# krea-ai/realtime-video

Measured on AMD Instinct MI355X. Metric: frames/sec at 832x480, 4-step 14B T2V (per-step DiT latency in config), higher is better.
Workload: dtype bf16

## Files before the change

### __graft_entry__.py

```python
import os
import sys

ROOT = os.path.dirname(os.path.abspath(__file__))
if ROOT not in sys.path:
    sys.path.insert(0, ROOT)


def build() -> None:
    from realtime_video_amd import _lib
    _lib.build(verbose=False)
    import realtime_video_amd.attention
    import realtime_video_amd.causal_model
    import realtime_video_amd.pipeline
    import realtime_video_amd.session
    import realtime_video_amd.taehv
    import realtime_video_amd.vae_decoder
    lib = _lib.load()
    missing = [s for s in _lib.declared_symbols() if not hasattr(lib, s)]
    if missing:
        raise RuntimeError(f"librtv_hip.so lacks symbols declared in include/rtv_hip.h: {missing}")
    import re
    import subprocess
    def audit(script, *argv, **env):
        r = subprocess.run([os.path.join(ROOT, "scripts", "micro", script), *argv], capture_output=True, text=True,
                           env=dict(os.environ, **env))
        return r.stdout + ("\n[stderr]\n" + r.stderr if r.stderr.strip() else "") + (f"\n[exit {r.returncode}]" if r.returncode else "")

    out = audit("w4_audit.sh", "600", W4_AUDIT_DIR=os.path.join(ROOT, "realtime_video_amd", "csrc", "build", "w4_audit"))
    ok = all(re.search(pat, out) for pat in (r"accumulation register outside asm: 0\b", r"v_accvgpr outside asm: 0\b", r"\bscratch 0\b",
                                              r"vgpr_spill_count: 0\b", r"private_segment_fixed_size: 0\b"))
    if not ok:
        raise RuntimeError("attn_w4 audit failed (scripts/micro/w4_audit.sh):\n" + out)
    out = audit("g5_audit.sh", G5_AUDIT_DIR=os.path.join(ROOT, "realtime_video_amd", "csrc", "build", "g5_audit"))
    if len(re.findall(r"AUDIT gemm5 F16=\d: vgpr_spills 0 private_segment 0 scratch_ops 0 mfma 120 compiler_acc_refs_before_last_accumulator_read 0 ", out)) != 2:
        raise RuntimeError("gemm5 audit failed (scripts/micro/g5_audit.sh):\n" + out)
    out = audit("h4_audit.sh", H4_AUDIT_DIR=os.path.join(ROOT, "realtime_video_amd", "csrc", "build", "h4_audit"))
    if len(re.findall(r"AUDIT _ZN3rtv1[78]conv_halo4p?_kernel\S*: arch_vgprs \d+ vgpr_spills 0 sgpr_spills \d+ private_segment 0 scratch_ops 0 "
                      r"mfma 216 compiler_acc_refs 0 \(a0-a7: 0\)", out)) != 2:
        raise RuntimeError("conv_halo4 audit failed (scripts/micro/h4_audit.sh):\n" + out)
    print(f"build ok: {_lib.LIB_PATH} ({len(_lib.declared_symbols())} C-ABI symbols; attn_w4 / gemm5 / conv_halo4 register audits clean)")


def smoke() -> None:
    import torch
    from oracle import vae_oracle as vo
    from oracle import wan_oracle as wo
    from realtime_video_amd.causal_model import CausalWanModel
# ... 46 lines not shown
```

### include/rtv_hip_lab.h

```cpp
#ifndef RTV_HIP_LAB_H
#define RTV_HIP_LAB_H
#ifdef __cplusplus
extern "C" {
#endif

int rtv_attn_set_waves(int waves);

int rtv_gemm_set_half_tail(int on);
int rtv_gemm_set_ragged_strips(int on);
int rtv_gemm_set_skip_idle(int on);
int rtv_conv_set_fuse_norm(int on);
int rtv_attn_set_skip_idle(int on);
int rtv_conv_set_halo(int on);
int rtv_dit_set_direct_v(int on);
int rtv_rope_set_wave(int mode);
int rtv_vae_set_fresh_tap_skip(int on);
int rtv_lab_build(void);

#ifdef __cplusplus
}
#endif
#endif
```

### realtime_video_amd/_lib.py

```python
import ctypes
import os
import subprocess

_HERE = os.path.dirname(os.path.abspath(__file__))
LIB_PATH = os.environ.get("RTV_LIB_PATH") or os.path.join(_HERE, "librtv_hip.so")
CSRC = os.path.join(_HERE, "csrc")

ABI_VERSION = 103

_lib = None

c_int, c_i64, c_f32, c_vp = ctypes.c_int, ctypes.c_int64, ctypes.c_float, ctypes.c_void_p

SIGNATURES = {
    "rtv_version": [],
    "rtv_quantize_fp8": [c_vp, c_i64, c_int, c_int, c_vp, c_i64, c_vp, c_vp, c_vp],
    "rtv_gemm_fp8": [c_vp, c_int, c_vp, c_int, c_vp, c_f32, c_vp, c_int, c_int, c_int, c_int, c_vp, c_int, c_vp, c_int,
                     c_int, c_int, c_vp, c_int, c_vp],
    "rtv_prof_enable": [c_int],
    "rtv_prof_read": [c_int, ctypes.POINTER(ctypes.c_double), ctypes.POINTER(c_i64),
                      ctypes.POINTER(ctypes.c_double)],
    "rtv_prof_reset": [],
    "rtv_prof_set_stride": [c_int, c_int],
    "rtv_prof_read_seen": [c_int, ctypes.POINTER(c_i64), ctypes.POINTER(ctypes.c_double)],
    "rtv_prof_bracket_overhead": [c_int, c_vp, ctypes.POINTER(ctypes.c_double)],
    "rtv_attn_fwd": [c_vp, c_vp, c_vp, c_vp, c_int, c_int, c_int, c_int, c_int,
                     c_i64, c_i64, c_i64, c_i64, c_i64, c_i64, c_i64, c_i64,
                     c_f32, c_int, c_int, c_int, c_vp],
    "rtv_attn_fwd_win": [c_vp, c_vp, c_vp, c_vp, c_int, c_int, c_int, c_int, c_int, c_int, c_int,
                         c_i64, c_i64, c_i64, c_i64, c_i64, c_i64, c_i64, c_i64,
                         c_f32, c_int, c_int, c_int, c_vp],
    "rtv_attn_fwd_dup": [c_vp, c_vp, c_vp, c_vp, c_int, c_int, c_int, c_int, c_int,
                         c_i64, c_i64, c_i64, c_i64, c_i64, c_i64, c_i64, c_i64,
                         c_f32, c_int, c_int, c_int, c_vp],
    "rtv_attn_fwd_split": [c_vp, c_vp, c_vp, c_vp, c_int, c_int, c_int, c_int, c_int, c_int, c_int,
                           c_i64, c_i64, c_i64, c_i64, c_i64, c_i64, c_i64, c_i64,
                           c_f32, c_int, c_int, c_int, c_vp, ctypes.c_size_t, c_int, c_vp],
    "rtv_attn_set_waves": [c_int],
    "rtv_attn_set_skip_idle": [c_int],
    "rtv_gemm_set_half_tail": [c_int],
    "rtv_gemm_set_skip_idle": [c_int],
    "rtv_gemm_set_ragged_strips": [c_int],
    "rtv_lab_build": [],
    "rtv_rope_set_wave": [c_int],
    "rtv_gemm": [c_vp, c_int, c_vp, c_int, c_vp, c_int, c_int, c_int, c_int,
                 c_vp, c_int, c_vp, c_int, c_int, c_int, c_vp, c_int, c_int, c_int, c_vp],
    "rtv_layernorm_modulate": [c_vp, c_vp, c_int, c_int, c_f32, c_vp, c_vp, c_int, c_int, c_int, c_vp, c_vp, c_vp],
    "rtv_rmsnorm": [c_vp, c_int, c_vp, c_int, c_int, c_int, c_f32, c_vp, c_vp],
    "rtv_qk_norm_rope_cache": [c_vp, c_vp, c_vp, c_vp, c_i64, c_int, c_int, c_int, c_int, c_f32,
                               c_vp, c_vp, c_vp, c_int, c_int, c_int, c_int, c_int, c_vp],
    "rtv_qk_norm_rope_cache_ring": [c_vp, c_vp, c_vp, c_vp, c_i64, c_int, c_int, c_int, c_int, c_f32,
                                    c_vp, c_vp, c_vp, c_int, c_int, c_int, c_int, c_int, c_int, c_int, c_int, c_vp],
    "rtv_modulation_table": [c_vp, c_vp, c_vp, c_int, c_int, c_int, c_int, c_int, c_vp],
    "rtv_sinusoidal_embedding": [c_vp, c_vp, c_int, c_int, c_vp],
# ... 79 lines not shown
```

### realtime_video_amd/csrc/attn_common.h

```cpp
#pragma once
#include "rtv_common.h"
#include "rtv_internal.h"

namespace rtv {

struct AttnParams {
  const uint16_t* q;
  const uint16_t* k;
  const uint16_t* v;
  uint16_t* o;
  int B, Lq, Lkv, H;
  int64_t q_bs, q_rs, k_bs, k_rs, v_bs, v_rs, o_bs, o_rs;
  float scale_log2e;
  int causal_block, q_offset;
  int n_qtiles;
  int n0, delta;
  int off0;
  int skip_idle;
  int dup_key;
  float dup_bias;
  int kv_splits;
  float* part_o;
  float* part_ml;
};

constexpr int ATT_D = 128;
constexpr int ATT_QW = 32;
constexpr int ATT_KT = 64;
constexpr int ATT_TILE_BYTES = ATT_KT * ATT_D * 2;

template <int V>
struct IntC {
  static constexpr int value = V;
};

template <bool F16>
// ... 76 lines not shown
```

### realtime_video_amd/csrc/attn_fwd.hip

```cpp
#include "attn_common.h"

namespace rtv {

#ifdef RTV_ATTN_TRACE
__device__ unsigned* g_attn_trace = nullptr;
#define ATT_STAMP(i)                                                                    \
  do {                                                                                  \
    if (tr_on && j >= 20 && j < 24) {                                                   \
      __builtin_amdgcn_sched_barrier(0);                                                \
      const unsigned t_ = (unsigned)__builtin_readcyclecounter();                       \
      if (lane == 0) tr_dst[(j - 20) * 6 + (i)] = t_;                                   \
      __builtin_amdgcn_sched_barrier(0);                                                \
    }                                                                                   \
  } while (0)
#else
#define ATT_STAMP(i)
#endif

template <bool F16>
__global__ __launch_bounds__(256) void attn_combine_kernel(const float* __restrict__ part_o, const float* __restrict__ part_ml,
                                                           uint16_t* __restrict__ o, int S, int B, int H, int Lq, int64_t o_bs,
                                                           int64_t o_rs) {
  const int64_t nrows = (int64_t)B * H * Lq;
  const int64_t row = (int64_t)blockIdx.x * 16 + (threadIdx.x >> 4);
// ... 583 lines not shown

using namespace rtv;

#ifdef RTV_ATTN_TRACE
extern "C" int rtv_attn_debug_trace(unsigned* buf) {
  return hipMemcpyToSymbol(HIP_SYMBOL(rtv::g_attn_trace), &buf, sizeof(buf)) == hipSuccess ? 0 : -1;
}
#endif

static std::atomic<int> g_attn_waves{0};
static std::atomic<bool> g_attn_lockstep{false};
static std::atomic<bool> g_attn_force_pp{false};
static std::atomic<bool> g_attn_skip_idle{true};
static std::atomic<int> g_attn_w4{-2};
constexpr int W4_DEFAULT = 600;
namespace rtv {
int launch_attn_w4(const AttnParams& p, bool f16, int variant, dim3 grid, hipStream_t stream);
}

extern "C" int rtv_attn_set_skip_idle(int on) {
  g_attn_skip_idle = on != 0;
  return 0;
}

extern "C" int rtv_attn_set_waves(int waves) {
  if (waves != 0 && waves != 4 && waves != 8 && waves != 81 && waves != 82 && !(waves >= 840 && waves <= 1639))
    return set_error(-1, "attn_set_waves: 0 (auto), 4, 8, 81 (256 rows, lockstep schedule), 82 (256 rows, four-phase schedule) or "
                         "840 + v (256 rows, one wave per SIMD, kernel variant v: attn_w4.hip)");
  g_attn_lockstep = waves == 81;
  g_attn_force_pp = waves == 82;
  g_attn_w4 = waves >= 840 ? waves - 840 : (waves == 81 || waves == 82 ? -1 : -2);
  g_attn_waves = waves > 8 ? 8 : waves;
// ... 96 lines not shown
  if (kv_splits > (Lkv + ATT_KT - 1) / ATT_KT) kv_splits = (Lkv + ATT_KT - 1) / ATT_KT;
  if (kv_splits < 1) kv_splits = 1;
  p.kv_splits = kv_splits;
  p.part_o = nullptr;
  p.part_ml = nullptr;
  if (kv_splits > 1) {
    if (dup_key >= 0) return set_error(-1, "attn_fwd: no KV split of a window with a counted key");
    const size_t rows = (size_t)kv_splits * B * H * Lq;
    if (!split_ws || ((uintptr_t)split_ws & 15) || split_ws_bytes < rows * (ATT_D + 2) * sizeof(float))
      return set_error(-1, "attn_fwd: split workspace missing, misaligned or too small (rtv_attn_split_workspace_bytes)");
    p.part_o = (float*)split_ws;
    p.part_ml = p.part_o + rows * ATT_D;
  }
  p.causal_block = causal_block;
  p.q_offset = q_offset;
  p.n0 = Lkv1 > 0 ? Lkv0 : Lkv;
  p.delta = Lkv1 > 0 ? seg1_row - Lkv0 : 0;
  int waves = g_attn_waves;
  const int cus = device_num_cus() > 0 ? device_num_cus() : 256;
  if (waves == 0) waves = ((int64_t)B * H * ((Lq + 255) / 256) * kv_splits < (int64_t)cus * 5 / 8 || Lkv <= 512) ? 4 : 8;
  const int qt_rows = ATT_QW * waves;
  p.n_qtiles = (Lq + qt_rows - 1) / qt_rows;
  const int lds = 4 * ATT_TILE_BYTES;
  const bool f16 = dtype == RTV_DTYPE_F16;
  const void* kerns[4] = {(const void*)attn_fwd_kernel<false, 8>, (const void*)attn_fwd_kernel<true, 8>,
                          (const void*)attn_fwd_kernel<false, 4>, (const void*)attn_fwd_kernel<true, 4>};
  static LdsAttr lds_attr[4];
  const int ki = (waves == 4 ? 2 : 0) + (f16 ? 1 : 0);
  if (int st = ensure_dynamic_lds(kerns[ki], lds, &lds_attr[ki], "attn_fwd")) return st;
  const int grid = B * H * p.n_qtiles;
// ... 19 lines not shown
    note_kernel(DK_ATTN_SPLIT_COMBINE);
    if (f16) hipLaunchKernelGGL((attn_combine_kernel<true>), cg, ct, 0, (hipStream_t)stream, p.part_o, p.part_ml, p.o, kv_splits, B, H, Lq, p.o_bs, p.o_rs);
    else hipLaunchKernelGGL((attn_combine_kernel<false>), cg, ct, 0, (hipStream_t)stream, p.part_o, p.part_ml, p.o, kv_splits, B, H, Lq, p.o_bs, p.o_rs);
    return check_launch("attn_combine");
  };
  p.off0 = 0;
  p.skip_idle = g_attn_skip_idle ? 1 : 0;
  const int base_shift = (Lkv1 > 0 && seg1_row < 0) ? seg1_row : 0;
  const int64_t top0 = (int64_t)p.n0 - base_shift, top1 = (int64_t)Lkv + p.delta - base_shift;
  const int64_t rs_max = k_row_stride > v_row_stride ? k_row_stride : v_row_stride;
  const bool offsets_fit = k_row_stride > 0 && v_row_stride > 0 &&
                           ((top0 > top1 ? top0 : top1) + ATT_KT) * rs_max * 2 < 0x7fffffffLL;
  int w4v = g_attn_w4;
  if (w4v == -2) w4v = Lkv >= 1024 ? W4_DEFAULT : -1;
  if (waves == 8 && w4v >= 0 && !f16 && Lkv1 == 0 && dup_key < 0 && offsets_fit) {
    if (int st = launch_attn_w4(p, f16, w4v, g, (hipStream_t)stream)) return st;
    note_kernel(DK_ATTN_W4);
    if (kv_splits > 1) return combine();
    return check_launch("attn_w4");
  }
  if (waves == 8 && !g_attn_lockstep && offsets_fit && dup_key < 0 && (Lkv >= 1024 || g_attn_force_pp)) {
    p.k += (int64_t)base_shift * k_row_stride;
    p.v += (int64_t)base_shift * v_row_stride;
    p.off0 = -base_shift;
    p.delta -= base_shift;
#ifdef RTV_ATTN_TRACE
    const int lds_pp = 2 * ATT_NB * ATT_TILE_BYTES + 256;
#else
    const int lds_pp = 2 * ATT_NB * ATT_TILE_BYTES;
#endif
    static LdsAttr pp_attr[2];
    const void* kp = f16 ? (const void*)attn_fwd_pp_kernel<true> : (const void*)attn_fwd_pp_kernel<false>;
// ... 19 lines not shown
```

### realtime_video_amd/csrc/attn_w4.hip

```cpp
#include "attn_common.h"

namespace rtv {
namespace w4 {

constexpr int NSLOT = 4;
constexpr int LDS_BYTES = 2 * NSLOT * ATT_TILE_BYTES;
constexpr int V_BASE = NSLOT * ATT_TILE_BYTES;
constexpr int QT = 256;
constexpr int QW = 64;

enum OpKind { OP_MAX = 0, OP_CMB, OP_XCH0, OP_XCH1, OP_DEC, OP_F, OP_E, OP_A, OP_CV, OP_SUM };
struct Op {
  int kind, qb, idx, sub, cost;
};
constexpr int N_PAIRS = 32;
constexpr int MAX_OPS = 300;
struct OpTable {
  Op op[MAX_OPS];
  int n;
};
template <bool RS>
constexpr OpTable make_ops() {
  OpTable t{};
  int n = 0;
// ... 169 lines not shown
  asm volatile("v_accvgpr_read_b32 %0, a[%c1]" : "=v"(r) : "n"(SRC));
  return r;
}
template <int REG>
__device__ __forceinline__ void acc_scale(float f) {
  float t;
  asm volatile("v_accvgpr_read_b32 %0, a[%c2]\n\ts_nop 0\n\tv_mul_f32 %0, %0, %1\n\ts_nop 0\n\tv_accvgpr_write_b32 a[%c2], %0" : "=&v"(t) : "v"(f), "n"(REG));
}
__device__ __forceinline__ void acc_settle() { asm volatile("s_nop 15\n\ts_nop 7" ); }

}

#ifdef RTV_LAB
__device__ unsigned long long* g_w4_probe = nullptr;
#endif

template <bool F16, int VARL>
__global__ __launch_bounds__(256, 1) void attn_fwd_w4_kernel(AttnParams p) {
  using namespace w4;
  constexpr int VAR = VARL % 10, LAB = (VARL / 10) % 10, OPT = VARL / 100;
  constexpr bool RS = OPT & 1, DMA_IMM = OPT & 2, EPI_LDS = OPT & 4;
  constexpr bool NO_VALU = LAB == 1 || LAB == 6, NO_EXP = LAB == 2, NO_FRAG = LAB == 3 || LAB == 6, NO_DMA = LAB == 4 || LAB == 6,
                 NO_WAIT = LAB == 5 || LAB == 6;
  using SC = Sched<VAR, RS>;
  using PB = PhaseB<RS>;
  constexpr int NB = PB::N;
  static_assert(SC::tab.ok, "softmax schedule violates the P^T hazard");
  extern __shared__ __attribute__((aligned(16))) char smem[];
  char* const sK = smem;
  char* const sV = smem + V_BASE;

  const int tid = threadIdx.x;
  const int lane = tid & 63;
  const int wave = __builtin_amdgcn_readfirstlane(tid >> 6);
  const int l31 = lane & 31, g = lane >> 5;

  int bh, qt;
  {
    const int nbh = p.B * p.H;
    const int bid = blockIdx.x;
    if (nbh % 8 == 0) {
      int xcd = bid & 7, slot = bid >> 3;
      bh = xcd + 8 * (slot / p.n_qtiles);
      qt = slot % p.n_qtiles;
    } else {
      bh = bid / p.n_qtiles;
      qt = bid % p.n_qtiles;
    }
  }
  const int b = bh / p.H, h = bh % p.H;
  const int q0 = qt * QT;
  const uint16_t* qb_ = p.q + (size_t)b * p.q_bs + (size_t)h * ATT_D;
  const uint16_t* kb = p.k + (size_t)b * p.k_bs + (size_t)h * ATT_D;
  const uint16_t* vb = p.v + (size_t)b * p.v_bs + (size_t)h * ATT_D;
  uint16_t* ob = p.o + (size_t)b * p.o_bs + (size_t)h * ATT_D;

  int q_row[2], kv_lim[2];
  int wave_min_lim = p.Lkv, wg_max_lim = p.Lkv;
#pragma unroll
  for (int qb = 0; qb < 2; ++qb) {
    q_row[qb] = q0 + wave * QW + qb * 32 + l31;
    kv_lim[qb] = p.Lkv;
  }
  if (p.causal_block > 0) {
// ... 3 lines not shown
    const int first = min(q0 + wave * QW, p.Lq - 1);
    wave_min_lim = min(p.Lkv, ((p.q_offset + first) / cb + 1) * cb);
    const int last = min(q0 + QT - 1, p.Lq - 1);
    wg_max_lim = min(p.Lkv, ((p.q_offset + last) / cb + 1) * cb);
  }
  wave_min_lim = __builtin_amdgcn_readfirstlane(wave_min_lim);
  const int ntiles = (wg_max_lim + ATT_KT - 1) / ATT_KT;
  int t_lo, t_hi;
  split_tile_range(p, ntiles, &t_lo, &t_hi);
  t_lo = __builtin_amdgcn_readfirstlane(t_lo);
  t_hi = __builtin_amdgcn_readfirstlane(t_hi);
  const int n_it = t_hi - t_lo;

  const int k_rs = __builtin_amdgcn_readfirstlane((int)p.k_rs), v_rs = __builtin_amdgcn_readfirstlane((int)p.v_rs);
  const int w_lkv = __builtin_amdgcn_readfirstlane(p.Lkv);
  const __amdgpu_buffer_rsrc_t rsrcK =
      __builtin_amdgcn_make_buffer_rsrc((void*)kb, 0, (int)((uint32_t)(w_lkv - 1) * (uint32_t)k_rs * 2u + 256u), 0x00020000);
  const __amdgpu_buffer_rsrc_t rsrcV =
      __builtin_amdgcn_make_buffer_rsrc((void*)vb, 0, (int)((uint32_t)(w_lkv - 1) * (uint32_t)v_rs * 2u + 256u), 0x00020000);
  const int t_last = (w_lkv - 1) / ATT_KT;
  const int st_row = wave * 16 + (lane >> 4);
  const int st_cp = lane & 15;
  uint32_t k_fast[4], v_fast[4];
#pragma unroll
  for (int i = 0; i < 4; ++i) {
    const int r = st_row + 4 * i;
    k_fast[i] = (uint32_t)(r * k_rs + (st_cp ^ (r & 15)) * 8) * 2u - (DMA_IMM ? 1024u * i : 0u);
    v_fast[i] = (uint32_t)(r * v_rs + (st_cp ^ ((r & 3) << 2)) * 8) * 2u - (DMA_IMM ? 1024u * i : 0u);
  }
  auto tile_soff = [&](int t, int rs) __attribute__((always_inline)) { return (uint32_t)(min(t, t_last) * ATT_KT * rs) * 2u; };
  const uint32_t lds_wave = (uint32_t)(uintptr_t)(RTV_LDS char*)smem + (uint32_t)wave * 4096u;
  auto piece = [&](auto vopc, auto slotc, auto ic, uint32_t lds_w, uint32_t soff) __attribute__((always_inline)) {
    constexpr int VOP = decltype(vopc)::value, SLOT = decltype(slotc)::value, I = decltype(ic)::value;
    constexpr int IMM = DMA_IMM ? I * 1024 : 0;
    RTV_LDS void* dst = (RTV_LDS void*)(uintptr_t)(lds_w + (uint32_t)(VOP * V_BASE + SLOT * ATT_TILE_BYTES + I * 1024 - IMM));
    if constexpr (VOP) __builtin_amdgcn_raw_ptr_buffer_load_lds(rsrcV, dst, 16, v_fast[I], soff, IMM, 0);
    else __builtin_amdgcn_raw_ptr_buffer_load_lds(rsrcK, dst, 16, k_fast[I], soff, IMM, 0);
  };
  auto stage_tile = [&](auto vopc, auto slotc, int t) __attribute__((always_inline)) {
    const uint32_t soff = tile_soff(t, decltype(vopc)::value ? v_rs : k_rs);
    static_for<0, 4>([&](auto ic) __attribute__((always_inline)) { piece(vopc, slotc, ic, lds_wave, soff); });
  };

  stage_tile(IntC<0>{}, IntC<0>{}, t_lo);
  stage_tile(IntC<0>{}, IntC<1>{}, t_lo + 1);
  stage_tile(IntC<0>{}, IntC<2>{}, t_lo + 2);
  stage_tile(IntC<1>{}, IntC<0>{}, t_lo);

  const bool idle_rows = p.skip_idle && q0 + wave * QW >= p.Lq;
  if (idle_rows) {
    asm volatile("s_waitcnt vmcnt(0)" ::: "memory");
    __builtin_amdgcn_s_barrier();
    auto idle_it = [&](auto cc, int i) __attribute__((always_inline)) {
      constexpr int C = decltype(cc)::value;
      stage_tile(IntC<0>{}, IntC<C>{}, t_lo + i + 4);
      stage_tile(IntC<1>{}, IntC<(C + 2) & 3>{}, t_lo + i + 2);
      asm volatile("s_waitcnt vmcnt(8)" ::: "memory");
      __builtin_amdgcn_s_barrier();
    };
    idle_it(IntC<3>{}, -1);
    for (int i = 0; i < n_it; i += 4) {
      idle_it(IntC<0>{}, i);
      if (i + 1 < n_it) idle_it(IntC<1>{}, i + 1);
      if (i + 2 < n_it) idle_it(IntC<2>{}, i + 2);
      if (i + 3 < n_it) idle_it(IntC<3>{}, i + 3);
    }
    asm volatile("s_waitcnt vmcnt(0)" ::: "memory");
    if (EPI_LDS && p.kv_splits <= 1) __syncthreads();
    return;
  }

  asm volatile("" ::: RTV_W4_ACC);
  {
    u32x4 qf[2][8];
#pragma unroll
    for (int qb = 0; qb < 2; ++qb) {
      const uint16_t* qp = qb_ + (size_t)min(q_row[qb], p.Lq - 1) * p.q_rs + g * 8;
#pragma unroll
      for (int dc = 0; dc < 8; ++dc) qf[qb][dc] = *(const u32x4*)(qp + dc * 16);
    }
    static_for<0, 64>([&](auto ic) __attribute__((always_inline)) {
      constexpr int i = decltype(ic)::value;
      acc_write<A_Q + i>(qf[i >> 5][(i >> 2) & 7][i & 3]);
    });
    static_for<0, 128>([&](auto ic) __attribute__((always_inline)) { acc_write<A_O + decltype(ic)::value>(0u); });
  }

  uint32_t k_rd32[8];
#pragma unroll
  for (int dc = 0; dc < 8; ++dc)
    k_rd32[dc] = (uint32_t)(uintptr_t)(RTV_LDS const char*)(sK + l31 * 256 + (((dc * 2 + g) ^ (l31 & 15)) << 4));
  const int i16 = lane & 15, h16 = (lane >> 4) & 1;
  uint32_t v_rd32[4];
#pragma unroll
  for (int db = 0; db < 4; ++db)
// ... 222 lines not shown
    uint32_t lds_w = lds_wave;
    asm volatile("" : "+s"(lds_w));
    phase_b(cc, IntC<1>{}, lds_w, tile_soff(t + 4, k_rs), tile_soff(t + 2, v_rs));
    rescale_o();
    end_of_iteration();
  };

  asm volatile("s_waitcnt vmcnt(0)" ::: "memory");
  __builtin_amdgcn_s_barrier();
  static_for<0, 16>([&](auto nc) __attribute__((always_inline)) {
    constexpr int n = decltype(nc)::value;
    lds_read128_a<A_KV + 4 * n, (n & 1) * 32 * 256>(k_rd32[n >> 1]);
  });
  lds_wait<0>();
  acc_settle();
  phase_a(IntC<3>{}, IntC<0>{});
  acc_settle();
  if ((t_lo + 1) * ATT_KT > wave_min_lim) mask_tile(IntC<0>{}, t_lo, false);
  phase_b(IntC<3>{}, IntC<0>{}, lds_wave, tile_soff(t_lo + 3, k_rs), tile_soff(t_lo + 1, v_rs));
  need_any = 0;
  end_of_iteration();

#ifdef RTV_LAB
  const unsigned long long probe_c0 = __builtin_readcyclecounter(), probe_r0 = __builtin_amdgcn_s_memrealtime();
#endif
  for (int i = 0; i < n_it; i += 4) {
    iteration(IntC<0>{}, i);
    if (i + 1 >= n_it) break;
    iteration(IntC<1>{}, i + 1);
    if (i + 2 >= n_it) break;
    iteration(IntC<2>{}, i + 2);
    if (i + 3 >= n_it) break;
    iteration(IntC<3>{}, i + 3);
  }
#ifdef RTV_LAB
  if (g_w4_probe != nullptr && wave == 0 && lane == 0 && blockIdx.x < 1024) {
    g_w4_probe[blockIdx.x * 3 + 0] = __builtin_readcyclecounter() - probe_c0;
    g_w4_probe[blockIdx.x * 3 + 1] = __builtin_amdgcn_s_memrealtime() - probe_r0;
    g_w4_probe[blockIdx.x * 3 + 2] = (unsigned long long)n_it;
  }
#endif
  asm volatile("s_waitcnt vmcnt(0)" ::: "memory");

  acc_settle();
  static_for<0, 2>([&](auto qc) __attribute__((always_inline)) {
    constexpr int qb = decltype(qc)::value;
    f32x16 oq[4];
    static_for<0, 64>([&](auto ic) __attribute__((always_inline)) {
      constexpr int i = decltype(ic)::value;
      oq[i >> 4][i & 15] = acc_read<A_O + qb * 64 + i>();
    });
    float l_tot;
    if constexpr (RS) l_tot = L[qb][0];
    else l_tot = l_run[qb] + __shfl_xor(l_run[qb], 32, 64);
    if (p.kv_splits > 1) {
      store_partial(p, bh, q_row[qb], g, oq, m_run[qb], l_tot);
    } else if constexpr (EPI_LDS) {
      const float inv = 1.0f / l_tot;
      char* img = smem + wave * (64 * 256);
      if constexpr (qb == 0) __syncthreads();
      const int row = qb * 32 + l31;
#pragma unroll
      for (int db = 0; db < 4; ++db)
#pragma unroll
        for (int i = 0; i < 4; ++i) {
          u32x2 w;
          w[0] = pack2<F16>(oq[db][4 * i + 0] * inv, oq[db][4 * i + 1] * inv);
          w[1] = pack2<F16>(oq[db][4 * i + 2] * inv, oq[db][4 * i + 3] * inv);
          *(u32x2*)(img + row * 256 + (((db * 4 + i) ^ (row & 15)) << 4) + g * 8) = w;
        }
      if constexpr (qb == 1) {
        asm volatile("s_waitcnt lgkmcnt(0)" ::: "memory");
        __builtin_amdgcn_sched_barrier(0);
        const int rsub = lane >> 4, cpos = lane & 15;
#pragma unroll
        for (int ps = 0; ps < 16; ++ps) {
          const int r = ps * 4 + rsub;
          const u32x4 t = *(const u32x4*)(img + r * 256 + ((cpos ^ (r & 15)) << 4));
          const int qr = q0 + wave * QW + r;
          if (qr < p.Lq) *(u32x4*)(ob + (size_t)qr * p.o_rs + cpos * 8) = t;
        }
      }
    } else {
      const float inv = 1.0f / l_tot;
      if (q_row[qb] < p.Lq) {
        uint16_t* op = ob + (size_t)q_row[qb] * p.o_rs + 4 * g;
#pragma unroll
        for (int db = 0; db < 4; ++db)
#pragma unroll
          for (int i = 0; i < 4; ++i) {
            u32x2 w;
            w[0] = pack2<F16>(oq[db][4 * i + 0] * inv, oq[db][4 * i + 1] * inv);
            w[1] = pack2<F16>(oq[db][4 * i + 2] * inv, oq[db][4 * i + 3] * inv);
            *(u32x2*)(op + db * 32 + i * 8) = w;
          }
      }
    }
  });
}

#ifdef RTV_LAB
}
extern "C" int rtv_attn_w4_probe(unsigned long long* buf) {
  return hipMemcpyToSymbol(HIP_SYMBOL(rtv::g_w4_probe), &buf, sizeof(buf)) == hipSuccess ? 0 : -1;
}
namespace rtv {
#endif

int launch_attn_w4(const AttnParams& p, bool f16, int variant, dim3 grid, hipStream_t stream) {
  static LdsAttr attr[800];
  if (variant < 0 || variant >= 800) return set_error(-1, "attn_w4: variant out of range");
  if (f16) return set_error(-1, "attn_w4: bf16 only (f16 launches stay on the four-phase kernel)");
#define RTV_W4_CASE(V)                                                                                        \
  case V: {                                                                                                   \
    const void* kp = (const void*)attn_fwd_w4_kernel<false, V>;                                               \
    if (int st = ensure_dynamic_lds(kp, w4::LDS_BYTES, &attr[V], "attn_w4")) return st;                       \
    hipLaunchKernelGGL((attn_fwd_w4_kernel<false, V>), grid, dim3(256), w4::LDS_BYTES, stream, p);            \
    break;                                                                                                    \
  }
  switch (variant) {
    RTV_W4_CASE(600)
    RTV_W4_CASE(200)
    RTV_W4_CASE(0)
#ifdef RTV_LAB
    RTV_W4_CASE(100)
    RTV_W4_CASE(300)
    RTV_W4_CASE(1)
    RTV_W4_CASE(2)
    RTV_W4_CASE(3)
    RTV_W4_CASE(101)
    RTV_W4_CASE(102)
    RTV_W4_CASE(103)
    RTV_W4_CASE(301)
    RTV_W4_CASE(302)
    RTV_W4_CASE(310)
    RTV_W4_CASE(320)
    RTV_W4_CASE(330)
    RTV_W4_CASE(340)
    RTV_W4_CASE(360)
#endif
    default:
      return set_error(-1, "attn_w4: variant = schedule (0..3) + 10 x lab experiment + 100 x options; this build has 200 and 0 "
                           "(lab build: more)");
  }
#undef RTV_W4_CASE
  return 0;
}

}
```

### realtime_video_amd/csrc/rtv_internal.h

```cpp
#pragma once
#include <hip/hip_runtime.h>

#include <atomic>

#include "../../include/rtv_hip.h"
#include "../../include/rtv_hip_lab.h"

namespace rtv {

int set_error(int code, const char* msg);
int check_launch(const char* what);

struct LdsAttr {
  std::atomic<uint64_t> done{0};
};
int ensure_dynamic_lds(const void* kernel, int bytes, LdsAttr* state, const char* what);

int device_num_cus();

enum ProfClass { PROF_GEMM = 0, PROF_ATTN, PROF_LN, PROF_ROPE, PROF_CONV, PROF_MISC, PROF_NCLASS };

struct ProfScope {
  ProfScope(int cls, hipStream_t stream, double work);
  ~ProfScope();
  int slot;
  hipStream_t stream;
};

enum DispatchKernel {
  DK_GEMM_128x128 = 0, DK_GEMM_OTHER_CFG, DK_GEMM8_256x256, DK_GEMM8M_128x256, DK_GEMM5_160x256, DK_GEMM_FP8_256x256,
  DK_ATTN_W4, DK_ATTN_FOUR_PHASE, DK_ATTN_LOCKSTEP_256ROW, DK_ATTN_LOCKSTEP_128ROW, DK_ATTN_SPLIT_COMBINE,
  DK_CONV_HALO4P, DK_CONV_HALO4, DK_CONV_HALO, DK_CONV_IGEMM, DK_COUNT
};
void note_kernel(int id);

struct GemmParams;
int launch_gemm(const GemmParams& p, int dtype, int tile_cfg, hipStream_t stream);
int launch_gemm8(const GemmParams& p, bool f16, bool split_k, hipStream_t stream);
int launch_gemm4(const GemmParams& p, bool f16, hipStream_t stream, int lab = 0);
int launch_gemm8m(const GemmParams& p, bool f16, bool split_k, hipStream_t stream);
int launch_gemm5(const GemmParams& p, bool f16, bool split_k, hipStream_t stream);
int launch_quantize_fp8(const uint16_t* x, int64_t ld, int M, int d, uint8_t* q, int64_t ldq, float* scale_out,
                        unsigned* amax_scratch, hipStream_t stream);
int launch_gemm_fp8(GemmParams p, const uint8_t* A, int lda, const uint8_t* W, int ldw, const float* a_scale, float w_scale,
                    hipStream_t stream);

int qk_norm_rope_check(int64_t cache_row_stride, int cache_row0, int M, int d, int num_heads, int F, int gh, int gw, int start_frame,
// ... 14 lines not shown
```

### realtime_video_amd/csrc/runtime.hip

```cpp
#include <mutex>
#include <string>
#include <vector>

#include "gemm_core.h"
#include "rtv_internal.h"

namespace rtv {

static thread_local std::string g_err;

int set_error(int code, const char* msg) {
  g_err = msg ? msg : "unknown error";
  if (code > 0) {
    g_err += ": ";
    g_err += hipGetErrorString((hipError_t)code);
  }
  return code == 0 ? -1 : code;
}

int ensure_dynamic_lds(const void* kernel, int bytes, LdsAttr* state, const char* what) {
  int dev = 0;
  if (hipGetDevice(&dev) != hipSuccess || dev < 0 || dev >= 64) return set_error(-1, "cannot query the current device");
  const uint64_t bit = 1ull << dev;
  if (state->done.load(std::memory_order_acquire) & bit) return 0;
// ... 11 lines not shown
  if (n == 0) {
    hipDeviceProp_t prop;
    if (hipGetDeviceProperties(&prop, dev) != hipSuccess) return 0;
    n = prop.multiProcessorCount;
    cus[dev].store(n, std::memory_order_relaxed);
  }
  return n;
}

static std::atomic<int64_t> g_dispatch[DK_COUNT];
static const char* const g_dispatch_names[DK_COUNT] = {
    "gemm_kernel<128x128>", "gemm_kernel<other tile config>", "gemm8_kernel<256x256 ping-pong>", "gemm8m_kernel<128x256 ping-pong>",
    "gemm5_kernel<160x256 one wave per SIMD>", "gemm_fp8_kernel<256x256>",
    "attn_fwd_w4_kernel<one wave per SIMD>", "attn_fwd_pp_kernel<four-phase>", "attn_fwd_kernel<lockstep, 256 rows>",
    "attn_fwd_kernel<lockstep, 128 rows>", "attn_combine_kernel<kv split>",
    "conv_halo4p_kernel<persistent>", "conv_halo4_kernel", "conv_halo_kernel", "conv_igemm_kernel"};
void note_kernel(int id) {
  if (id >= 0 && id < DK_COUNT) g_dispatch[id].fetch_add(1, std::memory_order_relaxed);
}

int check_launch(const char* what) {
  hipError_t e = hipGetLastError();
  if (e != hipSuccess) return set_error((int)e, what);
  return 0;
}

struct ProfRec {
  int cls;
  hipEvent_t start, stop;
  double work;
};
// ... 187 lines not shown
```

### realtime_video_amd/ops.py

```python
import ctypes
import math

import torch

from . import _lib

ACT_NONE, ACT_GELU_TANH, ACT_SILU = 0, 1, 2
DT_BF16, DT_F16 = 0, 1
PROF_CLASSES = {"gemm": 0, "attn": 1, "layernorm": 2, "rope": 3, "conv": 4, "misc": 5}


def _ptr(t):
    return ctypes.c_void_p(t.data_ptr()) if t is not None else ctypes.c_void_p(0)


def _stream():
    return ctypes.c_void_p(torch.cuda.current_stream().cuda_stream)


def _dt(t):
    if t.dtype == torch.bfloat16:
        return DT_BF16
    if t.dtype == torch.float16:
        return DT_F16
# ... 38 lines not shown
    if reset:
        lib.rtv_dispatch_reset.restype, lib.rtv_dispatch_reset.argtypes = ctypes.c_int, []
        lib.rtv_dispatch_reset()
    return out


def prof_read(cls):
    c = PROF_CLASSES[cls] if isinstance(cls, str) else int(cls)
    ms, n, work = ctypes.c_double(0), ctypes.c_int64(0), ctypes.c_double(0)
    _lib.call("rtv_prof_read", c, ctypes.byref(ms), ctypes.byref(n), ctypes.byref(work))
    sn, swork = ctypes.c_int64(0), ctypes.c_double(0)
    _lib.call("rtv_prof_read_seen", c, ctypes.byref(sn), ctypes.byref(swork))
    scale = swork.value / work.value if work.value > 0 else 1.0
    return {"ms": ms.value, "launches": n.value, "work": work.value, "seen_launches": sn.value, "seen_work": swork.value,
            "ms_class": ms.value * scale}


def attn_set_waves(waves=0):
    _lib.call("rtv_attn_set_waves", int(waves))


def attn_fwd(q, k, v, out=None, scale=None, causal_block=0, q_offset=0):
    _gpu(q, k, v)
    B, Lq, H, D = q.shape
    Lkv = k.shape[1]
    if k.shape != v.shape or k.shape[0] != B or k.shape[2] != H or k.shape[3] != D:
        raise ValueError(f"attention shape mismatch q{tuple(q.shape)} k{tuple(k.shape)} v{tuple(v.shape)}")
    if not (q.dtype == k.dtype == v.dtype):
        raise TypeError("q, k, v must share a dtype")
    for t in (q, k, v):
# ... 322 lines not shown
```

Measured before the change: 18.03.

## Add persistent attn_w4 kernel with next-unit prefetch and causal unit ordering

Adds a persistent form of the one-wave-per-SIMD attention kernel: the grid is capped at the CU count and each workgroup loops over (head, q-tile) units. While the epilogue of the current unit runs, it stages the next unit's first K/V tiles and Q fragments, overlapping the prologue with the previous tail. For causal launches it walks units in descending q-tile order with a serpentine pattern to balance the uneven causal work. It is on by default and adds a new kernel instantiation plus an audit, at the cost of more LDS reuse juggling and register pressure in the epilogue.

```diff
diff --git a/__graft_entry__.py b/__graft_entry__.py
--- a/__graft_entry__.py
+++ b/__graft_entry__.py
@@ -31,6 +31,12 @@
                                               r"vgpr_spill_count: 0\b", r"private_segment_fixed_size: 0\b"))
     if not ok:
         raise RuntimeError("attn_w4 audit failed (scripts/micro/w4_audit.sh):\n" + out)
+    out = audit("w4_audit.sh", "600", W4_KERNEL="attn_fwd_w4p_kernel",
+                W4_AUDIT_DIR=os.path.join(ROOT, "realtime_video_amd", "csrc", "build", "w4p_audit"))
+    ok = all(re.search(pat, out) for pat in (r"accumulation register outside asm: 0\b", r"v_accvgpr outside asm: 0\b", r"\bscratch 0\b",
+                                              r"vgpr_spill_count: 0\b", r"private_segment_fixed_size: 0\b", r"mfma 288\b"))
+    if not ok or re.search(r"vgpr_spill_count: [1-9]|private_segment_fixed_size: [1-9]", out):
+        raise RuntimeError("attn_w4 (persistent form) audit failed (scripts/micro/w4_audit.sh):\n" + out)
     out = audit("g5_audit.sh", G5_AUDIT_DIR=os.path.join(ROOT, "realtime_video_amd", "csrc", "build", "g5_audit"))
     if len(re.findall(r"AUDIT gemm5 F16=\d: vgpr_spills 0 private_segment 0 scratch_ops 0 mfma 120 compiler_acc_refs_before_last_accumulator_read 0 ", out)) != 2:
         raise RuntimeError("gemm5 audit failed (scripts/micro/g5_audit.sh):\n" + out)
diff --git a/include/rtv_hip_lab.h b/include/rtv_hip_lab.h
--- a/include/rtv_hip_lab.h
+++ b/include/rtv_hip_lab.h
@@ -5,6 +5,7 @@
 #endif
 
 int rtv_attn_set_waves(int waves);
+int rtv_attn_set_persistent(int persistent, int masked_unit_order);
 
 int rtv_gemm_set_half_tail(int on);
 int rtv_gemm_set_ragged_strips(int on);
diff --git a/realtime_video_amd/_lib.py b/realtime_video_amd/_lib.py
--- a/realtime_video_amd/_lib.py
+++ b/realtime_video_amd/_lib.py
@@ -38,6 +38,7 @@
                            c_f32, c_int, c_int, c_int, c_vp, ctypes.c_size_t, c_int, c_vp],
     "rtv_attn_set_waves": [c_int],
     "rtv_attn_set_skip_idle": [c_int],
+    "rtv_attn_set_persistent": [c_int, c_int],
     "rtv_gemm_set_half_tail": [c_int],
     "rtv_gemm_set_skip_idle": [c_int],
     "rtv_gemm_set_ragged_strips": [c_int],
diff --git a/realtime_video_amd/csrc/attn_common.h b/realtime_video_amd/csrc/attn_common.h
--- a/realtime_video_amd/csrc/attn_common.h
+++ b/realtime_video_amd/csrc/attn_common.h
@@ -20,6 +20,7 @@
   int dup_key;
   float dup_bias;
   int kv_splits;
+  int unit_order;
   float* part_o;
   float* part_ml;
 };
diff --git a/realtime_video_amd/csrc/attn_fwd.hip b/realtime_video_amd/csrc/attn_fwd.hip
--- a/realtime_video_amd/csrc/attn_fwd.hip
+++ b/realtime_video_amd/csrc/attn_fwd.hip
@@ -621,8 +621,18 @@
 static std::atomic<bool> g_attn_skip_idle{true};
 static std::atomic<int> g_attn_w4{-2};
 constexpr int W4_DEFAULT = 600;
+static std::atomic<int> g_attn_persistent{1};
+static std::atomic<int> g_attn_unit_order{-1};
 namespace rtv {
-int launch_attn_w4(const AttnParams& p, bool f16, int variant, dim3 grid, hipStream_t stream);
+int launch_attn_w4(const AttnParams& p, bool f16, int variant, dim3 grid, hipStream_t stream, int persistent_wgs);
+}
+
+extern "C" int rtv_attn_set_persistent(int persistent, int masked_unit_order) {
+  if (persistent < 0 || persistent > 1 || masked_unit_order < -1 || masked_unit_order > 2)
+    return set_error(-1, "attn_set_persistent: persistent 0 / 1, masked_unit_order -1 (by form), 0, 1 or 2");
+  g_attn_persistent = persistent;
+  g_attn_unit_order = masked_unit_order;
+  return 0;
 }
 
 extern "C" int rtv_attn_set_skip_idle(int on) {
@@ -749,6 +759,7 @@
   }
   p.causal_block = causal_block;
   p.q_offset = q_offset;
+  p.unit_order = 0;
   p.n0 = Lkv1 > 0 ? Lkv0 : Lkv;
   p.delta = Lkv1 > 0 ? seg1_row - Lkv0 : 0;
   int waves = g_attn_waves;
@@ -798,8 +809,11 @@
   int w4v = g_attn_w4;
   if (w4v == -2) w4v = Lkv >= 1024 ? W4_DEFAULT : -1;
   if (waves == 8 && w4v >= 0 && !f16 && Lkv1 == 0 && dup_key < 0 && offsets_fit) {
-    if (int st = launch_attn_w4(p, f16, w4v, g, (hipStream_t)stream)) return st;
-    note_kernel(DK_ATTN_W4);
+    const bool persist = g_attn_persistent != 0 && kv_splits == 1 && (w4v == 600 || w4v == 200);
+    const int order = g_attn_unit_order;
+    p.unit_order = causal_block > 0 ? (order >= 0 ? order : (persist ? 1 : 0)) : 0;
+    if (int st = launch_attn_w4(p, f16, w4v, g, (hipStream_t)stream, persist ? cus : 0)) return st;
+    note_kernel(persist ? DK_ATTN_W4_PERSISTENT : DK_ATTN_W4);
     if (kv_splits > 1) return combine();
     return check_launch("attn_w4");
   }
diff --git a/realtime_video_amd/csrc/attn_w4.hip b/realtime_video_amd/csrc/attn_w4.hip
--- a/realtime_video_amd/csrc/attn_w4.hip
+++ b/realtime_video_amd/csrc/attn_w4.hip
@@ -207,9 +207,13 @@
 #ifdef RTV_LAB
 __device__ unsigned long long* g_w4_probe = nullptr;
 #endif
-
-template <bool F16, int VARL>
-__global__ __launch_bounds__(256, 1) void attn_fwd_w4_kernel(AttnParams p) {
+#ifdef RTV_W4_TIMELINE
+__device__ unsigned long long* g_w4_timeline = nullptr;
+constexpr int W4_TIMELINE_UNITS = 4096;
+#endif
+
+template <bool F16, int VARL, bool PERSIST>
+__device__ __forceinline__ void attn_w4_body(const AttnParams& p) {
   using namespace w4;
   constexpr int VAR = VARL % 10, LAB = (VARL / 10) % 10, OPT = VARL / 100;
   constexpr bool RS = OPT & 1, DMA_IMM = OPT & 2, EPI_LDS = OPT & 4;
@@ -228,19 +232,38 @@
   const int wave = __builtin_amdgcn_readfirstlane(tid >> 6);
   const int l31 = lane & 31, g = lane >> 5;
 
+  const int nbh = p.B * p.H;
+  const bool xcd_groups = nbh % 8 == 0 && (!PERSIST || gridDim.x % 8 == 0);
+  const int grp_heads = xcd_groups ? nbh >> 3 : nbh;
+  const int grp_units = grp_heads * p.n_qtiles;
+  const int grp_j = xcd_groups ? (int)blockIdx.x >> 3 : (int)blockIdx.x, grp_nj = xcd_groups ? (int)gridDim.x >> 3 : (int)gridDim.x;
+  auto unit_at = [&](int r, int* bh_out, int* qt_out) __attribute__((always_inline)) -> bool {
+    int s = PERSIST ? r * grp_nj + ((p.unit_order == 1 && (r & 1)) ? grp_nj - 1 - grp_j : grp_j) : grp_j;
+    if (PERSIST && s >= grp_units) return false;
+    int hd, qt_;
+    if (p.unit_order == 1) {
+      hd = s % grp_heads;
+      qt_ = p.n_qtiles - 1 - s / grp_heads;
+    } else if (p.unit_order == 2) {
+      hd = s / p.n_qtiles;
+      qt_ = p.n_qtiles - 1 - s % p.n_qtiles;
+    } else {
+      hd = s / p.n_qtiles;
+      qt_ = s % p.n_qtiles;
+    }
+    *bh_out = xcd_groups ? ((int)blockIdx.x & 7) + 8 * hd : hd;
+    *qt_out = qt_;
+    return true;
+  };
+  int u_pos = 0;
+  u32x4 qf[2][8];
+  bool staged = false;
   int bh, qt;
-  {
-    const int nbh = p.B * p.H;
-    const int bid = blockIdx.x;
-    if (nbh % 8 == 0) {
-      int xcd = bid & 7, slot = bid >> 3;
-      bh = xcd + 8 * (slot / p.n_qtiles);
-      qt = slot % p.n_qtiles;
-    } else {
-      bh = bid / p.n_qtiles;
-      qt = bid % p.n_qtiles;
-    }
-  }
+  unit_at(0, &bh, &qt);
+  for (;;) {
+#ifdef RTV_W4_TIMELINE
+  const unsigned long long tl_start = __builtin_amdgcn_s_memrealtime();
+#endif
   const int b = bh / p.H, h = bh % p.H;
   const int q0 = qt * QT;
   const uint16_t* qb_ = p.q + (size_t)b * p.q_bs + (size_t)h * ATT_D;
@@ -274,10 +297,10 @@
 
   const int k_rs = __builtin_amdgcn_readfirstlane((int)p.k_rs), v_rs = __builtin_amdgcn_readfirstlane((int)p.v_rs);
   const int w_lkv = __builtin_amdgcn_readfirstlane(p.Lkv);
-  const __amdgpu_buffer_rsrc_t rsrcK =
-      __builtin_amdgcn_make_buffer_rsrc((void*)kb, 0, (int)((uint32_t)(w_lkv - 1) * (uint32_t)k_rs * 2u + 256u), 0x00020000);
-  const __amdgpu_buffer_rsrc_t rsrcV =
-      __builtin_amdgcn_make_buffer_rsrc((void*)vb, 0, (int)((uint32_t)(w_lkv - 1) * (uint32_t)v_rs * 2u + 256u), 0x00020000);
+  auto make_rsrc = [&](const uint16_t* base, int rs) __attribute__((always_inline)) {
+    return __builtin_amdgcn_make_buffer_rsrc((void*)base, 0, (int)((uint32_t)(w_lkv - 1) * (uint32_t)rs * 2u + 256u), 0x00020000);
+  };
+  __amdgpu_buffer_rsrc_t rsrcK = make_rsrc(kb, k_rs), rsrcV = make_rsrc(vb, v_rs);
   const int t_last = (w_lkv - 1) / ATT_KT;
   const int st_row = wave * 16 + (lane >> 4);
   const int st_cp = lane & 15;
@@ -302,10 +325,37 @@
     static_for<0, 4>([&](auto ic) __attribute__((always_inline)) { piece(vopc, slotc, ic, lds_wave, soff); });
   };
 
-  stage_tile(IntC<0>{}, IntC<0>{}, t_lo);
-  stage_tile(IntC<0>{}, IntC<1>{}, t_lo + 1);
-  stage_tile(IntC<0>{}, IntC<2>{}, t_lo + 2);
-  stage_tile(IntC<1>{}, IntC<0>{}, t_lo);
+  auto stage_prologue = [&](int t0) __attribute__((always_inline)) {
+    stage_tile(IntC<0>{}, IntC<0>{}, t0);
+    stage_tile(IntC<0>{}, IntC<1>{}, t0 + 1);
+    stage_tile(IntC<0>{}, IntC<2>{}, t0 + 2);
+    stage_tile(IntC<1>{}, IntC<0>{}, t0);
+  };
+  auto load_q = [&](const uint16_t* qbase, int row0) __attribute__((always_inline)) {
+#pragma unroll
+    for (int qb = 0; qb < 2; ++qb) {
+      const uint16_t* qp = qbase + (size_t)min(row0 + wave * QW + qb * 32 + l31, p.Lq - 1) * p.q_rs + g * 8;
+#pragma unroll
+      for (int dc = 0; dc < 8; ++dc) qf[qb][dc] = *(const u32x4*)(qp + dc * 16);
+    }
+  };
+  if (!PERSIST || !staged) stage_prologue(t_lo);
+  int nx_bh = 0, nx_qt = 0;
+  bool has_next = false;
+  auto stage_next = [&]() __attribute__((always_inline)) {
+    if constexpr (PERSIST) {
+      int r = u_pos + 1;
+      asm volatile("" : "+s"(r));
+      has_next = unit_at(r, &nx_bh, &nx_qt);
+      if (has_next) {
+        const int nb = nx_bh / p.H, nh = nx_bh % p.H;
+        rsrcK = make_rsrc(p.k + (size_t)nb * p.k_bs + (size_t)nh * ATT_D, k_rs);
+        rsrcV = make_rsrc(p.v + (size_t)nb * p.v_bs + (size_t)nh * ATT_D, v_rs);
+        stage_prologue(0);
+        load_q(p.q + (size_t)nb * p.q_bs + (size_t)nh * ATT_D, nx_qt * QT);
+      }
+    }
+  };
 
   const bool idle_rows = p.skip_idle && q0 + wave * QW >= p.Lq;
   if (idle_rows) {
@@ -326,19 +376,22 @@
       if (i + 3 < n_it) idle_it(IntC<3>{}, i + 3);
     }
     asm volatile("s_waitcnt vmcnt(0)" ::: "memory");
-    if (EPI_LDS && p.kv_splits <= 1) __syncthreads();
-    return;
+    stage_next();
+    if (EPI_LDS && p.kv_splits <= 1) {
+      if constexpr (PERSIST) __builtin_amdgcn_s_barrier();
+      else __syncthreads();
+    }
+    if (!has_next) return;
+    bh = nx_bh;
+    qt = nx_qt;
+    ++u_pos;
+    staged = true;
+    continue;
   }
 
   asm volatile("" ::: RTV_W4_ACC);
   {
-    u32x4 qf[2][8];
-#pragma unroll
-    for (int qb = 0; qb < 2; ++qb) {
-      const uint16_t* qp = qb_ + (size_t)min(q_row[qb], p.Lq - 1) * p.q_rs + g * 8;
-#pragma unroll
-      for (int dc = 0; dc < 8; ++dc) qf[qb][dc] = *(const u32x4*)(qp + dc * 16);
-    }
+    if (!PERSIST || !staged) load_q(qb_, q0);
     static_for<0, 64>([&](auto ic) __attribute__((always_inline)) {
       constexpr int i = decltype(ic)::value;
       acc_write<A_Q + i>(qf[i >> 5][(i >> 2) & 7][i & 3]);
@@ -591,6 +644,9 @@
   });
   lds_wait<0>();
   acc_settle();
+#ifdef RTV_W4_TIMELINE
+  const unsigned long long tl_first = __builtin_amdgcn_s_memrealtime();
+#endif
   phase_a(IntC<3>{}, IntC<0>{});
   acc_settle();
   if ((t_lo + 1) * ATT_KT > wave_min_lim) mask_tile(IntC<0>{}, t_lo, false);
@@ -617,8 +673,14 @@
     g_w4_probe[blockIdx.x * 3 + 2] = (unsigned long long)n_it;
   }
 #endif
+#ifdef RTV_W4_TIMELINE
+  const unsigned long long tl_loop = __builtin_amdgcn_s_memrealtime();
+#endif
   asm volatile("s_waitcnt vmcnt(0)" ::: "memory");
-
+  stage_next();
+
+  int lane_e = lane;
+  if constexpr (PERSIST) asm volatile("" : "+v"(lane_e));
   acc_settle();
   static_for<0, 2>([&](auto qc) __attribute__((always_inline)) {
     constexpr int qb = decltype(qc)::value;
@@ -634,9 +696,13 @@
       store_partial(p, bh, q_row[qb], g, oq, m_run[qb], l_tot);
     } else if constexpr (EPI_LDS) {
       const float inv = 1.0f / l_tot;
-      char* img = smem + wave * (64 * 256);
-      if constexpr (qb == 0) __syncthreads();
-      const int row = qb * 32 + l31;
+      char* img = PERSIST ? smem + (wave == 0 ? 3 * ATT_TILE_BYTES : V_BASE + wave * ATT_TILE_BYTES) : smem + wave * (64 * 256);
+      if constexpr (qb == 0) {
+        if constexpr (PERSIST) __builtin_amdgcn_s_barrier();
+        else __syncthreads();
+      }
+      const int row = qb * 32 + (lane_e & 31), ge = lane_e >> 5;
+      const uint32_t img32 = (uint32_t)(uintptr_t)(RTV_LDS char*)img;
 #pragma unroll
       for (int db = 0; db < 4; ++db)
 #pragma unroll
@@ -644,18 +710,38 @@
           u32x2 w;
           w[0] = pack2<F16>(oq[db][4 * i + 0] * inv, oq[db][4 * i + 1] * inv);
           w[1] = pack2<F16>(oq[db][4 * i + 2] * inv, oq[db][4 * i + 3] * inv);
-          *(u32x2*)(img + row * 256 + (((db * 4 + i) ^ (row & 15)) << 4) + g * 8) = w;
+          const int off = row * 256 + (((db * 4 + i) ^ (row & 15)) << 4) + ge * 8;
+          if constexpr (PERSIST) asm volatile("ds_write_b64 %0, %1" ::"v"(img32 + (uint32_t)off), "v"(w) : "memory");
+          else *(u32x2*)(img + off) = w;
         }
       if constexpr (qb == 1) {
         asm volatile("s_waitcnt lgkmcnt(0)" ::: "memory");
         __builtin_amdgcn_sched_barrier(0);
-        const int rsub = lane >> 4, cpos = lane & 15;
-#pragma unroll
-        for (int ps = 0; ps < 16; ++ps) {
-          const int r = ps * 4 + rsub;
-          const u32x4 t = *(const u32x4*)(img + r * 256 + ((cpos ^ (r & 15)) << 4));
-          const int qr = q0 + wave * QW + r;
-          if (qr < p.Lq) *(u32x4*)(ob + (size_t)qr * p.o_rs + cpos * 8) = t;
+        const int rsub = lane_e >> 4, cpos = lane_e & 15;
+        if constexpr (PERSIST) {
+#pragma unroll
+          for (int ps = 0; ps < 16; ps += 4) {
+            u32x4 t[4];
+#pragma unroll
+            for (int j = 0; j < 4; ++j) {
+              const int r = (ps + j) * 4 + rsub;
+              t[j] = lds_read128_at<0>(img32 + (uint32_t)(r * 256 + ((cpos ^ (r & 15)) << 4)));
+            }
+            asm volatile("s_waitcnt lgkmcnt(0)" : "+v"(t[0]), "+v"(t[1]), "+v"(t[2]), "+v"(t[3]));
+#pragma unroll
+            for (int j = 0; j < 4; ++j) {
+              const int qr = q0 + wave * QW + (ps + j) * 4 + rsub;
+              if (qr < p.Lq) *(u32x4*)(ob + (size_t)qr * p.o_rs + cpos * 8) = t[j];
+            }
+          }
+        } else {
+#pragma unroll
+          for (int ps = 0; ps < 16; ++ps) {
+            const int r = ps * 4 + rsub;
+            const u32x4 t = *(const u32x4*)(img + r * 256 + ((cpos ^ (r & 15)) << 4));
+            const int qr = q0 + wave * QW + r;
+            if (qr < p.Lq) *(u32x4*)(ob + (size_t)qr * p.o_rs + cpos * 8) = t;
+          }
         }
       }
     } else {
@@ -674,6 +760,37 @@
       }
     }
   });
+#ifdef RTV_W4_TIMELINE
+  if (g_w4_timeline != nullptr && wave == 0 && lane == 0) {
+    const int uid = bh * p.n_qtiles + qt;
+    if (uid < W4_TIMELINE_UNITS && blockIdx.y == 0) {
+      unsigned long long* r = g_w4_timeline + (size_t)uid * 8;
+      r[0] = __builtin_amdgcn_s_getreg((31 << 11) | 20);
+      r[1] = __builtin_amdgcn_s_getreg((31 << 11) | 4);
+      r[2] = tl_start;
+      r[3] = tl_first;
+      r[4] = tl_loop;
+      r[5] = __builtin_amdgcn_s_memrealtime();
+      r[6] = (unsigned long long)n_it;
+      r[7] = (unsigned long long)u_pos;
+    }
+  }
+#endif
+  if (!has_next) break;
+  bh = nx_bh;
+  qt = nx_qt;
+  ++u_pos;
+  staged = true;
+  }
+}
+
+template <bool F16, int VARL>
+__global__ __launch_bounds__(256, 1) void attn_fwd_w4_kernel(AttnParams p) {
+  attn_w4_body<F16, VARL, false>(p);
+}
+template <bool F16, int VARL>
+__global__ __launch_bounds__(256, 1) void attn_fwd_w4p_kernel(AttnParams p) {
+  attn_w4_body<F16, VARL, true>(p);
 }
 
 #ifdef RTV_LAB
@@ -684,20 +801,40 @@
 namespace rtv {
 #endif
 
-int launch_attn_w4(const AttnParams& p, bool f16, int variant, dim3 grid, hipStream_t stream) {
-  static LdsAttr attr[800];
+#ifdef RTV_W4_TIMELINE
+}
+extern "C" int rtv_attn_w4_timeline(unsigned long long* buf) {
+  return hipMemcpyToSymbol(HIP_SYMBOL(rtv::g_w4_timeline), &buf, sizeof(buf)) == hipSuccess ? 0 : -1;
+}
+namespace rtv {
+#endif
+
+int launch_attn_w4(const AttnParams& p, bool f16, int variant, dim3 grid, hipStream_t stream, int persistent_wgs) {
+  static LdsAttr attr[800], attr_p[800];
   if (variant < 0 || variant >= 800) return set_error(-1, "attn_w4: variant out of range");
   if (f16) return set_error(-1, "attn_w4: bf16 only (f16 launches stay on the four-phase kernel)");
+  const bool persist = persistent_wgs > 0 && grid.y == 1 && p.kv_splits <= 1 && (variant == 600 || variant == 200);
+  if (persist && grid.x > (unsigned)persistent_wgs) grid.x = (unsigned)persistent_wgs;
+#define RTV_W4_LAUNCH(KERN, V, ATTR)                                                                          \
+  {                                                                                                           \
+    const void* kp = (const void*)KERN<false, V>;                                                             \
+    if (int st = ensure_dynamic_lds(kp, w4::LDS_BYTES, &ATTR[V], "attn_w4")) return st;                       \
+    hipLaunchKernelGGL((KERN<false, V>), grid, dim3(256), w4::LDS_BYTES, stream, p);                          \
+  }
 #define RTV_W4_CASE(V)                                                                                        \
   case V: {                                                                                                   \
-    const void* kp = (const void*)attn_fwd_w4_kernel<false, V>;                                               \
-    if (int st = ensure_dynamic_lds(kp, w4::LDS_BYTES, &attr[V], "attn_w4")) return st;                       \
-    hipLaunchKernelGGL((attn_fwd_w4_kernel<false, V>), grid, dim3(256), w4::LDS_BYTES, stream, p);            \
+    RTV_W4_LAUNCH(attn_fwd_w4_kernel, V, attr)                                                                \
     break;                                                                                                    \
   }
+#define RTV_W4_CASE_P(V)                                                                                      \
+  case V: {                                                                                                   \
+    if (persist) RTV_W4_LAUNCH(attn_fwd_w4p_kernel, V, attr_p)                                                \
+    else RTV_W4_LAUNCH(attn_fwd_w4_kernel, V, attr)                                                           \
+    break;                                                                                                    \
+  }
   switch (variant) {
-    RTV_W4_CASE(600)
-    RTV_W4_CASE(200)
+    RTV_W4_CASE_P(600)
+    RTV_W4_CASE_P(200)
     RTV_W4_CASE(0)
 #ifdef RTV_LAB
     RTV_W4_CASE(100)
@@ -721,6 +858,8 @@
                            "(lab build: more)");
   }
 #undef RTV_W4_CASE
+#undef RTV_W4_CASE_P
+#undef RTV_W4_LAUNCH
   return 0;
 }
 
diff --git a/realtime_video_amd/csrc/rtv_internal.h b/realtime_video_amd/csrc/rtv_internal.h
--- a/realtime_video_amd/csrc/rtv_internal.h
+++ b/realtime_video_amd/csrc/rtv_internal.h
@@ -30,7 +30,7 @@
 enum DispatchKernel {
   DK_GEMM_128x128 = 0, DK_GEMM_OTHER_CFG, DK_GEMM8_256x256, DK_GEMM8M_128x256, DK_GEMM5_160x256, DK_GEMM_FP8_256x256,
   DK_ATTN_W4, DK_ATTN_FOUR_PHASE, DK_ATTN_LOCKSTEP_256ROW, DK_ATTN_LOCKSTEP_128ROW, DK_ATTN_SPLIT_COMBINE,
-  DK_CONV_HALO4P, DK_CONV_HALO4, DK_CONV_HALO, DK_CONV_IGEMM, DK_COUNT
+  DK_CONV_HALO4P, DK_CONV_HALO4, DK_CONV_HALO, DK_CONV_IGEMM, DK_ATTN_W4_PERSISTENT, DK_COUNT
 };
 void note_kernel(int id);
 
diff --git a/realtime_video_amd/csrc/runtime.hip b/realtime_video_amd/csrc/runtime.hip
--- a/realtime_video_amd/csrc/runtime.hip
+++ b/realtime_video_amd/csrc/runtime.hip
@@ -49,7 +49,8 @@
     "gemm5_kernel<160x256 one wave per SIMD>", "gemm_fp8_kernel<256x256>",
     "attn_fwd_w4_kernel<one wave per SIMD>", "attn_fwd_pp_kernel<four-phase>", "attn_fwd_kernel<lockstep, 256 rows>",
     "attn_fwd_kernel<lockstep, 128 rows>", "attn_combine_kernel<kv split>",
-    "conv_halo4p_kernel<persistent>", "conv_halo4_kernel", "conv_halo_kernel", "conv_igemm_kernel"};
+    "conv_halo4p_kernel<persistent>", "conv_halo4_kernel", "conv_halo_kernel", "conv_igemm_kernel",
+    "attn_fwd_w4p_kernel<one wave per SIMD, persistent>"};
 void note_kernel(int id) {
   if (id >= 0 && id < DK_COUNT) g_dispatch[id].fetch_add(1, std::memory_order_relaxed);
 }
diff --git a/realtime_video_amd/ops.py b/realtime_video_amd/ops.py
--- a/realtime_video_amd/ops.py
+++ b/realtime_video_amd/ops.py
@@ -76,6 +76,10 @@
     scale = swork.value / work.value if work.value > 0 else 1.0
     return {"ms": ms.value, "launches": n.value, "work": work.value, "seen_launches": sn.value, "seen_work": swork.value,
             "ms_class": ms.value * scale}
+
+
+def attn_set_persistent(persistent=1, masked_unit_order=-1):
+    _lib.call("rtv_attn_set_persistent", int(persistent), int(masked_unit_order))
 
 
 def attn_set_waves(waves=0):
```

Result: no change. 18.07 (median of 6 runs) (+0.2%).
